# twndus/YelpRecommendation

Hardware: NVIDIA B200
Metric: ngcf_bpr_train_triples_per_sec (higher is better)
Workload: dtype f32

## Files before the change

### yelprecommendation_b200/csrc/common.cuh

```cuda
#pragma once
#include <cuda_runtime.h>
#include <cooperative_groups.h>
#include <stdint.h>
#include "../../include/yelprec_b200.h"

namespace cg = cooperative_groups;

#define YR_CHECK_LAUNCH()                                   \
  do {                                                      \
    cudaError_t e__ = cudaGetLastError();                   \
    if (e__ != cudaSuccess) return (int)e__;                \
  } while (0)

#define YR_CUDA(call)                                       \
  do {                                                      \
    cudaError_t e__ = (call);                               \
    if (e__ != cudaSuccess) return (int)e__;                \
  } while (0)

int yr_eval_exact_launch(const float* Uemb, int64_t nU, const float* Vt, int64_t ldt, int64_t nI, int d,
                         const int64_t* eval_uid, int64_t n_eval, const int32_t* mask_ptr,
                         const int32_t* mask_idx, const int32_t* act_ptr, const int32_t* act_idx,
                         const int32_t* act_nuniq, const double* inv_log2, int K, int64_t* topk_out,
                         float* topk_score, double* user_metrics, int32_t* err, const int32_t* row_list,
                         const int32_t* n_rows_dev, yr_stream stream, void* ws = nullptr, size_t ws_bytes = 0);
int yr_eval_reduce_launch(const double* user_metrics, const int32_t* act_ptr, const int32_t* act_nuniq,
                          int64_t n_eval, double* metric_sums, yr_stream stream);

int yr_ngcf_dense_fwd_tc_launch_d(int d, const float* E, const float* LE, const float* W1, const float* W2, float slope,
                                  int64_t n, float* Eout, cudaStream_t s, const int32_t* row_list = nullptr,
                                  const int32_t* row_count = nullptr, int64_t row_cap = 0, int reserve_sms = 0);
int yr_ngcf_dense_bwd_tc_launch(int d, const float* E, const float* LE, const float* En, const float* Gn, const float* W1,
                                const float* W2, float slope, int64_t n, float* G, float* T, float* ws, int* n_parts,
                                cudaStream_t s, const int32_t* row_list = nullptr, const int32_t* row_count = nullptr,
                                int64_t row_cap = 0, int reserve_sms = 0);
int yr_spmm_csr_rows(const yr_csr* A, int d, const float* X, float* Y, const int32_t* row_flag, cudaStream_t s);

namespace yr {

constexpr int kWarp = 32;
constexpr unsigned kFull = 0xffffffffu;

__device__ __forceinline__ float warp_sum(float v) {
#pragma unroll
  for (int o = 16; o > 0; o >>= 1) v += __shfl_xor_sync(kFull, v, o);
  return v;
}
__device__ __forceinline__ double warp_sum_d(double v) {
#pragma unroll
  for (int o = 16; o > 0; o >>= 1) v += __shfl_xor_sync(kFull, v, o);
  return v;
}

__device__ __forceinline__ void grid_sync(cg::grid_group& grid) {
  __syncwarp();
  grid.sync();
  __syncwarp();
}

template <int VPL> struct Row { float x[VPL]; };

template <int VPL>
__device__ __forceinline__ Row<VPL> ld_row(const float* __restrict__ row, int lane) {
  Row<VPL> r;
  if constexpr (VPL == 1) {
    r.x[0] = row[lane];
  } else if constexpr (VPL == 2) {
    float2 t = reinterpret_cast<const float2*>(row)[lane];
    r.x[0] = t.x; r.x[1] = t.y;
  } else {
#pragma unroll
    for (int j = 0; j < VPL / 4; ++j) {
      float4 t = reinterpret_cast<const float4*>(row)[j * 32 + lane];
      r.x[4 * j + 0] = t.x; r.x[4 * j + 1] = t.y; r.x[4 * j + 2] = t.z; r.x[4 * j + 3] = t.w;
    }
  }
  return r;
}

template <int VPL>
__device__ __forceinline__ Row<VPL> ld_row_cg(const float* __restrict__ row, int lane) {
  Row<VPL> r;
  if constexpr (VPL == 1) {
    r.x[0] = __ldcg(row + lane);
  } else if constexpr (VPL == 2) {
    float2 t = __ldcg(reinterpret_cast<const float2*>(row) + lane);
    r.x[0] = t.x; r.x[1] = t.y;
  } else {
// ... 151 lines not shown
```

### yelprecommendation_b200/csrc/ngcf.cu

```cuda
#include <stdlib.h>
#include "common.cuh"

namespace yr {

__device__ __forceinline__ void fma2(float2& acc, float a, const float2 b) { acc = __ffma2_rn(make_float2(a, a), b, acc); }

template <int D>
struct DenseCfg {
  static constexpr int kThreads = 256;
  static constexpr int kColGroups = D / 4;
  static constexpr int kRowGroups = kThreads / kColGroups;
  static constexpr int TM = 4 * kRowGroups;
  static constexpr int RO = D / kRowGroups;
  static constexpr size_t kSmemFwd = (size_t)(2 * D * TM + 2 * D * D) * sizeof(float);
  static constexpr size_t kSmemBwd = (size_t)(3 * TM * D + 2 * D * D) * sizeof(float);
  static_assert(D == 32 || D == 64 || D == 128, "dense transforms: D in {32, 64, 128}");
};

template <int D>
__global__ void __launch_bounds__(256)
ngcf_dense_fwd_kernel(const float* __restrict__ E, const float* __restrict__ LE,
                      const float* __restrict__ W1, const float* __restrict__ W2, float slope,
                      int64_t n, float* __restrict__ Eout) {
  using C = DenseCfg<D>;
// ... 406 lines not shown
                                 float* E_next, cudaStream_t s) {
  using C = DenseCfg<D>;
  static AttrOnce attr;
  { int rc_ = attr.set(ngcf_dense_fwd_kernel<D>, (int)C::kSmemFwd); if (rc_) return rc_; }
  const int64_t n_tiles = (n + C::TM - 1) / C::TM;
  int64_t grid = (int64_t)yr_sm_count() * (D <= 64 ? 3 : 1);
  if (grid > n_tiles) grid = n_tiles;
  ngcf_dense_fwd_kernel<D><<<(unsigned)grid, C::kThreads, C::kSmemFwd, s>>>(E, LE, W1, W2, slope, n, E_next);
  YR_CHECK_LAUNCH();
  return YR_OK;
}

template <int D>
static int dense_bwd_fp32_launch(int64_t n, const float* E, const float* LE, const float* E_next, const float* G_next,
                                 const float* W1, const float* W2, float slope, float* G, float* T, float* ws,
                                 cudaStream_t s, int* n_parts) {
  using C = DenseCfg<D>;
  static AttrOnce attr;
  { int rc_ = attr.set(ngcf_dense_bwd_kernel<D>, (int)C::kSmemBwd); if (rc_) return rc_; }
  const int64_t n_tiles = (n + C::TM - 1) / C::TM;
  int64_t grid = (int64_t)yr_sm_count() * (D <= 64 ? kBwdCtasPerSm : 1);
  if (grid > n_tiles) grid = n_tiles;
  ngcf_dense_bwd_kernel<D><<<(unsigned)grid, C::kThreads, C::kSmemBwd, s>>>(E, LE, E_next, G_next, W1, W2, slope, n, G, T, ws,
                                                                          nullptr, nullptr);
  YR_CHECK_LAUNCH();
  *n_parts = (int)grid;
  return YR_OK;
}

extern "C" int yr_ngcf_dense_fwd(int d, int64_t n, const float* E, const float* LE, const float* W1, const float* W2,
                                 float slope, float* E_next, int dense_mode, yr_stream stream) {
  if (!E || !LE || !W1 || !W2 || !E_next || n < 0 || !mode_ok(dense_mode)) return YR_ERR_BAD_ARG;
  if (d != 32 && d != 64 && d != 128) return YR_ERR_BAD_DIM;
  if (n == 0) return YR_OK;
  if (fwd_tc(dense_mode) && (d == 64 || d == 128))
    return yr_ngcf_dense_fwd_tc_launch_d(d, E, LE, W1, W2, slope, n, E_next, (cudaStream_t)stream, nullptr, nullptr, 0,
                                         reserve_of(dense_mode));
  switch (d) {
    case 32: return dense_fwd_fp32_launch<32>(n, E, LE, W1, W2, slope, E_next, (cudaStream_t)stream);
    case 64: return dense_fwd_fp32_launch<64>(n, E, LE, W1, W2, slope, E_next, (cudaStream_t)stream);
    default: return dense_fwd_fp32_launch<128>(n, E, LE, W1, W2, slope, E_next, (cudaStream_t)stream);
  }
}

extern "C" int yr_ngcf_layer_fwd(const yr_csr* L, int d, const float* E, const float* W1, const float* W2,
                                 float slope, float* E_next, float* LE_save, int dense_mode, yr_stream stream) {
  if (!L || !E || !W1 || !W2 || !E_next || !LE_save || L->n_rows <= 0 || !mode_ok(dense_mode)) return YR_ERR_BAD_ARG;
  if (d != 32 && d != 64 && d != 128) return YR_ERR_BAD_DIM;
  int rc = yr_spmm_csr(L, d, E, LE_save, 0, stream);
  if (rc) return rc;
  return yr_ngcf_dense_fwd(d, L->n_rows, E, LE_save, W1, W2, slope, E_next, dense_mode, stream);
}

extern "C" size_t yr_ngcf_layer_bwd_ws_bytes(int d) {
  return (size_t)yr_sm_count() * kBwdCtasPerSm * 2 * (size_t)d * d * sizeof(float);
}

static int dense_bwd_launch(int d, int64_t n, const float* E, const float* LE, const float* E_next, const float* G_next,
                            const float* W1, const float* W2, float slope, float* G, float* T, void* ws, size_t ws_bytes,
                            int dense_mode, cudaStream_t s, int* n_parts) {
  if (!E || !LE || !E_next || !G_next || !W1 || !W2 || !G || !T || !ws || n <= 0 || !mode_ok(dense_mode)) return YR_ERR_BAD_ARG;
  if (d != 32 && d != 64 && d != 128) return YR_ERR_BAD_DIM;
  if (ws_bytes < yr_ngcf_layer_bwd_ws_bytes(d)) return YR_ERR_WORKSPACE;
  if (bwd_tc(dense_mode) && (d == 64 || d == 128))
    return yr_ngcf_dense_bwd_tc_launch(d, E, LE, E_next, G_next, W1, W2, slope, n, G, T, (float*)ws, n_parts, s, nullptr, nullptr,
                                       0, reserve_of(dense_mode));
  switch (d) {
    case 32: return dense_bwd_fp32_launch<32>(n, E, LE, E_next, G_next, W1, W2, slope, G, T, (float*)ws, s, n_parts);
    case 64: return dense_bwd_fp32_launch<64>(n, E, LE, E_next, G_next, W1, W2, slope, G, T, (float*)ws, s, n_parts);
    default: return dense_bwd_fp32_launch<128>(n, E, LE, E_next, G_next, W1, W2, slope, G, T, (float*)ws, s, n_parts);
  }
}

static int dense_bwd_reduce(int d, const void* ws, int n_parts, float* dW1, float* dW2, cudaStream_t s) {
  const int len = 2 * d * d;
  reduce_partials_kernel<<<(len + 31) / 32, 256, 0, s>>>((const float*)ws, n_parts, len, dW1, dW2, d * d);
  YR_CHECK_LAUNCH();
  return YR_OK;
}

extern "C" int yr_ngcf_dense_bwd(int d, int64_t n, const float* E, const float* LE, const float* E_next,
                                 const float* G_next, const float* W1, const float* W2, float slope,
                                 float* G, float* T, float* dW1, float* dW2, void* ws, size_t ws_bytes,
                                 int dense_mode, yr_stream stream) {
  if (!dW1 || !dW2) return YR_ERR_BAD_ARG;
  int parts = 0;
  int rc = dense_bwd_launch(d, n, E, LE, E_next, G_next, W1, W2, slope, G, T, ws, ws_bytes, dense_mode, (cudaStream_t)stream,
                            &parts);
  if (rc) return rc;
  return dense_bwd_reduce(d, ws, parts, dW1, dW2, (cudaStream_t)stream);
}

namespace yr {
__global__ void __launch_bounds__(256)
touched_rows_kernel(const int64_t* __restrict__ uid, const int64_t* __restrict__ pos, const int64_t* __restrict__ neg,
                    int64_t B, int64_t nU, int64_t nI, int32_t* flag, int32_t* list, int32_t* count) {
  for (int64_t i = (int64_t)blockIdx.x * blockDim.x + threadIdx.x; i < 3 * B; i += (int64_t)gridDim.x * blockDim.x) {
    const int which = (int)(i / B);
    const int64_t b = i - which * B;
    const int64_t id = which == 0 ? uid[b] : (which == 1 ? pos[b] : neg[b]);
    if (id < 0 || id >= (which == 0 ? nU : nI)) continue;
    const int64_t row = which == 0 ? id : nU + id;
    if (atomicExch(flag + row, 1) == 0) list[atomicAdd(count, 1)] = (int32_t)row;
  }
}

__global__ void __launch_bounds__(256)
untouch_rows_kernel(int32_t* flag, const int32_t* __restrict__ list, const int32_t* __restrict__ count) {
  const int n = *count;
  for (int i = blockIdx.x * blockDim.x + threadIdx.x; i < n; i += gridDim.x * blockDim.x) flag[list[i]] = 0;
}

template <int D>
__global__ void __launch_bounds__(256)
spmm_scatter_rows_kernel(yr_csr A, const int32_t* __restrict__ flag, const float* __restrict__ T, float* __restrict__ G) {
  constexpr int kVec = D / 4, LPR = kVec >= 32 ? 32 : kVec, VPT = kVec / LPR, CPW = 32 / LPR;
  const int lane = threadIdx.x & 31, sub = lane / LPR, sl = lane % LPR;
  const int gwarp = (blockIdx.x * blockDim.x + threadIdx.x) >> 5;
  const int nwarps = (gridDim.x * blockDim.x) >> 5;
// ... 2 lines not shown
    const int c = cb + sub;
    int4 dsc = make_int4(0, 0, 0, -1);
    if (c < A.n_chunks) dsc = __ldg(desc + c);
    const int row = dsc.x, s0 = dsc.y;
    int len = dsc.z & 0xff;
    if (c >= A.n_chunks || !__ldg(flag + row)) len = 0;
    int maxlen = len;
#pragma unroll
    for (int o = LPR; o < 32; o <<= 1) maxlen = max(maxlen, __shfl_xor_sync(kFull, maxlen, o));
    if (maxlen == 0) continue;
    float4 t[VPT];
#pragma unroll
    for (int v = 0; v < VPT; ++v)
      t[v] = len ? reinterpret_cast<const float4*>(T + (int64_t)row * D)[sl * VPT + v] : make_float4(0.f, 0.f, 0.f, 0.f);
    for (int j0 = 0; j0 < maxlen; j0 += LPR) {
      const int j = j0 + sl;
      const int cc = (j < len) ? __ldg(A.col + s0 + j) : -1;
      const float aa = (j < len) ? __ldg(A.val + s0 + j) : 0.f;
      for (int q = 0; q < LPR && j0 + q < maxlen; ++q) {
        const int cq = __shfl_sync(kFull, cc, q, LPR);
        const float a = __shfl_sync(kFull, aa, q, LPR);
        if (cq >= 0) {
#pragma unroll
          for (int v = 0; v < VPT; ++v)
            atomicAdd(reinterpret_cast<float4*>(G + (int64_t)cq * D) + sl * VPT + v,
                      make_float4(a * t[v].x, a * t[v].y, a * t[v].z, a * t[v].w));
        }
      }
    }
  }
}
}

struct SideStream { cudaStream_t stream; cudaEvent_t fork, join; };
static SideStream* side_stream() {
  static SideStream pool[64];
  static int state[64];
  const char* e = getenv("YR_NGCF_SIDE_STREAM");
  if (e && e[0] == '0') return nullptr;
  int dev = 0;
  if (cudaGetDevice(&dev) != cudaSuccess || dev < 0 || dev >= 64) return nullptr;
  if (state[dev] == 0) {
    SideStream& x = pool[dev];
    const bool ok = cudaStreamCreateWithFlags(&x.stream, cudaStreamNonBlocking) == cudaSuccess &&
                    cudaEventCreateWithFlags(&x.fork, cudaEventDisableTiming) == cudaSuccess &&
                    cudaEventCreateWithFlags(&x.join, cudaEventDisableTiming) == cudaSuccess;
    state[dev] = ok ? 1 : -1;
  }
  return state[dev] == 1 ? &pool[dev] : nullptr;
}

static int rows_reduce(const yr_ngcf_state* st, int l, int parts, cudaStream_t s, SideStream* side);

static int ngcf_layer_bwd_rows(const yr_ngcf_state* st, int l, float slope, cudaStream_t s, SideStream* side) {
  const int d = st->d;
  using C = DenseCfg<64>;
  if (d != 64) return YR_ERR_BAD_DIM;
  if (bwd_tc(st->dense_mode) && st->row_list_cap >= 16384) {
    int parts = 0;
    int rc = yr_ngcf_dense_bwd_tc_launch(d, st->E[l], st->LE[l], st->E[l + 1], st->G[l + 1], st->W1[l], st->W2[l], slope,
                                         st->nU + st->nI, st->G[l], st->T, (float*)st->ws, &parts, s, st->row_list,
                                         st->row_count, st->row_list_cap);
    if (rc) return rc;
    rc = rows_reduce(st, l, parts, s, side);
    if (rc) return rc;
    const int64_t blocks_tc = ((int64_t)st->L.n_chunks + 15) / 16;
    spmm_scatter_rows_kernel<64><<<(unsigned)blocks_tc, 256, 0, s>>>(st->L, st->row_flag, st->T, st->G[l]);
    YR_CHECK_LAUNCH();
    return YR_OK;
  }
  int64_t grid = (st->row_list_cap + C::TM - 1) / C::TM;
  const int64_t cap = (int64_t)yr_sm_count() * kBwdCtasPerSm;
  if (grid > cap) grid = cap;
  if (grid < 1) grid = 1;
  static AttrOnce attr;
  { int rc_ = attr.set(ngcf_dense_bwd_kernel<64>, (int)C::kSmemBwd); if (rc_) return rc_; }
  ngcf_dense_bwd_kernel<64><<<(unsigned)grid, C::kThreads, C::kSmemBwd, s>>>(
      st->E[l], st->LE[l], st->E[l + 1], st->G[l + 1], st->W1[l], st->W2[l], slope, st->nU + st->nI, st->G[l], st->T,
      (float*)st->ws, st->row_list, st->row_count);
  YR_CHECK_LAUNCH();
  int rc = rows_reduce(st, l, (int)grid, s, side);
  if (rc) return rc;
  const int wpb = 8, cpw = 2;
  int64_t blocks = ((int64_t)st->L.n_chunks + wpb * cpw - 1) / (wpb * cpw);
  spmm_scatter_rows_kernel<64><<<(unsigned)blocks, 256, 0, s>>>(st->L, st->row_flag, st->T, st->G[l]);
  YR_CHECK_LAUNCH();
  return YR_OK;
}

static int rows_reduce(const yr_ngcf_state* st, int l, int parts, cudaStream_t s, SideStream* side) {
  const int len = 2 * st->d * st->d;
  cudaStream_t rs = s;
  if (side) {
    YR_CUDA(cudaEventRecord(side->fork, s));
    YR_CUDA(cudaStreamWaitEvent(side->stream, side->fork, 0));
    rs = side->stream;
  }
  reduce_partials_kernel<<<(len + 31) / 32, 256, 0, rs>>>((const float*)st->ws, parts, len, st->dW1[l], st->dW2[l],
                                                         st->d * st->d);
  YR_CHECK_LAUNCH();
  if (side) YR_CUDA(cudaEventRecord(side->join, side->stream));
  return YR_OK;
}

extern "C" int yr_ngcf_layer_bwd(const yr_csr* LT, int d, const float* E, const float* LE, const float* E_next,
                                 const float* G_next, const float* W1, const float* W2, float slope,
                                 float* G, float* T, float* dW1, float* dW2, void* ws, size_t ws_bytes,
                                 int dense_mode, yr_stream stream) {
  if (!LT || LT->n_rows <= 0) return YR_ERR_BAD_ARG;
  int rc = yr_ngcf_dense_bwd(d, LT->n_rows, E, LE, E_next, G_next, W1, W2, slope, G, T, dW1, dW2, ws, ws_bytes, dense_mode,
                             stream);
  if (rc) return rc;
  return yr_spmm_csr(LT, d, T, G, 1, stream);
// ... 96 lines not shown
  if (rc) return rc;
  if (n_prefix < 0 || n_prefix > st->n_layers) return YR_ERR_BAD_ARG;
  for (int l = 0; l < n_prefix; ++l) {
    rc = yr_ngcf_layer_fwd(&st->L, st->d, st->E[l], st->W1[l], st->W2[l], slope, st->E[l + 1], st->LE[l], st->dense_mode,
                           stream);
    if (rc) return rc;
  }
  return YR_OK;
}

extern "C" int yr_ngcf_propagate(const yr_ngcf_state* st, float slope, yr_stream stream) {
  int rc = ngcf_state_ok(st);
  if (rc) return rc;
  for (int l = 0; l < st->n_layers; ++l) {
    rc = yr_ngcf_layer_fwd(&st->L, st->d, st->E[l], st->W1[l], st->W2[l], slope,
                           st->E[l + 1], st->LE[l], st->dense_mode, stream);
    if (rc) return rc;
  }
  return YR_OK;
}

extern "C" int yr_ngcf_train_step_ex(const yr_ngcf_state* st, const yr_opt* opt, float slope,
                                     const int64_t* uid, const int64_t* pos, const int64_t* neg, int64_t B,
                                     float* step_loss, int prefix_done, yr_stream stream);

extern "C" int yr_ngcf_train_step(const yr_ngcf_state* st, const yr_opt* opt, float slope,
                                  const int64_t* uid, const int64_t* pos, const int64_t* neg, int64_t B,
                                  float* step_loss, yr_stream stream) {
  return yr_ngcf_train_step_ex(st, opt, slope, uid, pos, neg, B, step_loss, 0, stream);
}

static int train_step_body(const yr_ngcf_state* st, const yr_opt* opt, float slope,
                           const int64_t* uid, const int64_t* pos, const int64_t* neg, int64_t B,
                           float* step_loss, int prefix_done, yr_stream stream, bool* rows_armed) {
  int rc = ngcf_state_ok(st);
  if (rc) return rc;
  if (prefix_done < 0 || prefix_done > st->n_layers) return YR_ERR_BAD_ARG;
  if (!opt || !uid || !pos || !neg || B <= 0 || yr_csr_ok(&st->LT) || !st->T ||
      !st->E_dev || !st->G_dev || !st->ws || !st->loss)
    return YR_ERR_BAD_ARG;
  if (opt->kind < YR_OPT_SGD || opt->kind > YR_OPT_ADAMW) return YR_ERR_BAD_OPT;
  const int L = st->n_layers, d = st->d;
  const int64_t n = st->nU + st->nI;
  cudaStream_t s = (cudaStream_t)stream;
  SideStream* side = side_stream();
  for (int l = 0; l <= L; ++l)
    if (!st->G[l]) return YR_ERR_BAD_ARG;
  cudaStream_t ms = side ? side->stream : s;
  if (side) {
    YR_CUDA(cudaEventRecord(side->fork, s));
    YR_CUDA(cudaStreamWaitEvent(side->stream, side->fork, 0));
  }
  for (int l = 0; l <= L; ++l) YR_CUDA(cudaMemsetAsync(st->G[l], 0, sizeof(float) * (size_t)n * d, ms));
  const bool rows_path = st->row_flag && st->row_list && st->row_count && st->row_list_cap >= 3 * B && d == 64 &&
                         st->top_rows_mode != 0;
  if (rows_path) {
    touched_rows_kernel<<<(unsigned)((3 * B + 255) / 256), 256, 0, ms>>>(uid, pos, neg, B, st->nU, st->nI, st->row_flag,
                                                                        st->row_list, st->row_count);
    YR_CHECK_LAUNCH();
    *rows_armed = true;
  }
  if (side) YR_CUDA(cudaEventRecord(side->join, side->stream));
  if (rows_path && fwd_tc(st->dense_mode)) {
    for (int l = (prefix_done < L - 1 ? prefix_done : L - 1); l + 1 < L; ++l) {
      rc = yr_ngcf_layer_fwd(&st->L, d, st->E[l], st->W1[l], st->W2[l], slope, st->E[l + 1], st->LE[l], st->dense_mode,
                           stream);
      if (rc) return rc;
    }
    if (side) YR_CUDA(cudaStreamWaitEvent(s, side->join, 0));
    rc = yr_spmm_csr_rows(&st->L, d, st->E[L - 1], st->LE[L - 1], st->row_flag, s);
    if (rc) return rc;
    rc = yr_ngcf_dense_fwd_tc_launch_d(d, st->E[L - 1], st->LE[L - 1], st->W1[L - 1], st->W2[L - 1], slope, n, st->E[L], s,
                                       st->row_list, st->row_count, 3 * B);
    if (rc) return rc;
  } else {
    for (int l = prefix_done; l < L; ++l) {
      rc = yr_ngcf_layer_fwd(&st->L, d, st->E[l], st->W1[l], st->W2[l], slope, st->E[l + 1], st->LE[l], st->dense_mode,
                           stream);
      if (rc) return rc;
    }
  }
  if (side) YR_CUDA(cudaStreamWaitEvent(s, side->join, 0));
  rc = yr_ngcf_tail(st->E_dev, st->G_dev, L, st->nU, st->nI, d, uid, pos, neg, B, nullptr, nullptr, st->loss,
                    step_loss, st->err, stream);
  if (rc) return rc;
  bool reduce_pending = false;
  for (int l = L - 1; l >= 0; --l) {
    if (!st->dW1[l] || !st->dW2[l]) return YR_ERR_BAD_ARG;
    if (rows_path && l == L - 1) {
      rc = ngcf_layer_bwd_rows(st, l, slope, s, side);
      if (rc) return rc;
      reduce_pending = side != nullptr;
      cudaStream_t us = s;
      if (side) {
        YR_CUDA(cudaStreamWaitEvent(s, side->join, 0));
        reduce_pending = false;
        YR_CUDA(cudaEventRecord(side->fork, s));
        YR_CUDA(cudaStreamWaitEvent(side->stream, side->fork, 0));
        us = side->stream;
      }
      untouch_rows_kernel<<<(unsigned)((3 * B + 255) / 256), 256, 0, us>>>(st->row_flag, st->row_list, st->row_count);
      YR_CHECK_LAUNCH();
      YR_CUDA(cudaMemsetAsync(st->row_count, 0, sizeof(int32_t), us));
      *rows_armed = false;
      continue;
    }
    if (side && reduce_pending) { YR_CUDA(cudaStreamWaitEvent(s, side->join, 0)); reduce_pending = false; }
    int parts = 0;
    rc = dense_bwd_launch(d, n, st->E[l], st->LE[l], st->E[l + 1], st->G[l + 1], st->W1[l], st->W2[l], slope, st->G[l],
                          st->T, st->ws, st->ws_bytes, st->dense_mode, s, &parts);
    if (rc) return rc;
    if (side) {
      YR_CUDA(cudaEventRecord(side->fork, s));
      YR_CUDA(cudaStreamWaitEvent(side->stream, side->fork, 0));
      rc = dense_bwd_reduce(d, st->ws, parts, st->dW1[l], st->dW2[l], side->stream);
      if (rc) return rc;
      YR_CUDA(cudaEventRecord(side->join, side->stream));
      reduce_pending = true;
    } else {
      rc = dense_bwd_reduce(d, st->ws, parts, st->dW1[l], st->dW2[l], s);
      if (rc) return rc;
    }
    rc = yr_spmm_csr(&st->LT, d, st->T, st->G[l], 1, stream);
    if (rc) return rc;
  }
  if (side && reduce_pending) YR_CUDA(cudaStreamWaitEvent(s, side->join, 0));
  float *pp[2 * YR_NGCF_MAX_LAYERS + 1], *gg[2 * YR_NGCF_MAX_LAYERS + 1], *mm[2 * YR_NGCF_MAX_LAYERS + 1],
      *vv[2 * YR_NGCF_MAX_LAYERS + 1];
  int64_t nn[2 * YR_NGCF_MAX_LAYERS + 1];
  int cnt = 0;
  pp[cnt] = st->E[0]; gg[cnt] = st->G[0]; mm[cnt] = st->mE; vv[cnt] = st->vE; nn[cnt++] = n * d;
  for (int l = 0; l < L; ++l) {
    pp[cnt] = st->W1[l]; gg[cnt] = st->dW1[l]; mm[cnt] = st->mW1[l]; vv[cnt] = st->vW1[l]; nn[cnt++] = (int64_t)d * d;
    pp[cnt] = st->W2[l]; gg[cnt] = st->dW2[l]; mm[cnt] = st->mW2[l]; vv[cnt] = st->vW2[l]; nn[cnt++] = (int64_t)d * d;
  }
  for (int c0 = 0; c0 < cnt; c0 += YR_OPT_MAX_TENSORS) {
    const int c = (cnt - c0 < YR_OPT_MAX_TENSORS) ? cnt - c0 : YR_OPT_MAX_TENSORS;
    rc = yr_dense_opt_step_multi(c, pp + c0, gg + c0, mm + c0, vv + c0, nn + c0, opt, 0, stream);
    if (rc) return rc;
  }
  return YR_OK;
}

extern "C" int yr_ngcf_train_step_ex(const yr_ngcf_state* st, const yr_opt* opt, float slope,
                                     const int64_t* uid, const int64_t* pos, const int64_t* neg, int64_t B,
                                     float* step_loss, int prefix_done, yr_stream stream) {
  bool rows_armed = false;
  const int rc = train_step_body(st, opt, slope, uid, pos, neg, B, step_loss, prefix_done, stream, &rows_armed);
  if (rc == YR_OK) return rc;
  cudaStream_t s = (cudaStream_t)stream;
  if (SideStream* side = side_stream()) {
    if (cudaEventRecord(side->join, side->stream) == cudaSuccess) cudaStreamWaitEvent(s, side->join, 0);
  }
  if (rows_armed && st && st->row_flag && st->row_list && st->row_count) {
    untouch_rows_kernel<<<(unsigned)((3 * B + 255) / 256), 256, 0, s>>>(st->row_flag, st->row_list, st->row_count);
    cudaMemsetAsync(st->row_count, 0, sizeof(int32_t), s);
  }
  return rc;
}

extern "C" int yr_ngcf_concat(const float* const* E_layers, int n_layers, int64_t n, int d, float* out,
                              yr_stream stream) {
  if (!E_layers || !out || n <= 0 || d <= 0 || (d & 3) || n_layers < 0 || n_layers > YR_NGCF_MAX_LAYERS)
// ... 9 lines not shown
```

### yelprecommendation_b200/csrc/ngcf_tc_bwd.cu

```cuda
#include <stdlib.h>
#include "tc_common.cuh"

namespace yr {

constexpr int kBwdThreads = 416;
constexpr int kBwdTM = 128;
constexpr int kFlushTiles = 4;

__device__ __forceinline__ uint32_t mn_off(int mn, int k, uint32_t lbo, uint32_t sbo) {
  return (uint32_t)(k >> 2) * sbo + (uint32_t)(mn >> 5) * lbo + (uint32_t)(k & 3) * 128u +
         ((((uint32_t)(mn & 31) >> 3) ^ (uint32_t)(k & 3)) << 5) + (uint32_t)(mn & 7) * 4u;
}
__device__ __forceinline__ uint64_t mn_desc(uint32_t smem_addr, uint32_t lbo, uint32_t sbo) {
  uint64_t d = 0;
  d |= (uint64_t)((smem_addr & 0x3FFFFu) >> 4);
  d |= (uint64_t)((lbo >> 4) & 0x3FFFu) << 16;
  d |= (uint64_t)((sbo >> 4) & 0x3FFFu) << 32;
  d |= (uint64_t)1 << 46;
  d |= (uint64_t)1 << 61;
  return d;
}
__device__ __forceinline__ void mbar_expect_tx_b(uint64_t* bar, uint32_t bytes) {
  asm volatile("mbarrier.expect_tx.relaxed.cta.shared::cta.b64 [%0], %1;" ::"r"(s2u(bar)), "r"(bytes) : "memory");
}
__device__ __forceinline__ void bulk_g2s_b(void* dst, const void* src, uint32_t bytes, uint64_t* bar) {
  asm volatile("cp.async.bulk.shared::cluster.global.mbarrier::complete_tx::bytes [%0], [%1], %2, [%3];" ::"r"(s2u(dst)),
               "l"(src), "r"(bytes), "r"(s2u(bar))
               : "memory");
}

template <int D>
struct BwdTc {
  static_assert(D == 64 || D == 128, "tensor-core backward: d in {64, 128}");
  static constexpr int kSlabs = D / 32;
  static constexpr int kXG = D == 128 ? 2 : 1;
  static constexpr int kHalves = D / 64;
  static constexpr uint32_t kBlk = 16384;
  static constexpr uint32_t kPair = 2 * kBlk;
  static constexpr uint32_t kStage = (1 + kXG) * kPair;
  static constexpr int kNst = D == 128 ? 2 : 3;
  static constexpr uint32_t kRing = kNst * kStage;
  static constexpr uint32_t kEpiOff = kRing;
  static constexpr uint32_t kEpiBytes = 4 * 32 * 256;
  static constexpr uint32_t kBarOff = kEpiOff + kEpiBytes;
  static constexpr size_t kSmem = (size_t)kBarOff + 256 + 1024;
  static constexpr int kAcc = D == 128 ? 1 : 2;
  static constexpr uint32_t kAccCols = D == 128 ? 256 : 128;
  static constexpr uint32_t kTmemCols = 512;
  static constexpr uint32_t kColG2 = 256;
  static constexpr uint32_t kSboW = 2048, kSboSP = 2048, kSboZ = (D / 32) * 512, kLbo = 512;
  static constexpr int kItems = kSlabs + 4 * kHalves;
  static constexpr size_t kWsplitBytes = (size_t)kSlabs * kXG * kPair;
};

template <int D>
__global__ void __launch_bounds__(256)
ngcf_split_weights_bwd_kernel(const float* __restrict__ W1, const float* __restrict__ W2, unsigned char* __restrict__ ws) {
  using C = BwdTc<D>;
  const int total = 2 * D * (D / 4);
  for (int idx = blockIdx.x * blockDim.x + threadIdx.x; idx < total; idx += gridDim.x * blockDim.x) {
    const int X = idx / (D * (D / 4)), rem = idx % (D * (D / 4));
    const int o = rem / (D / 4), c4 = rem % (D / 4), j = o >> 5, k = o & 31;
    float4 hi, lo;
    split4(__ldg(reinterpret_cast<const float4*>((X ? W2 : W1) + o * D) + c4), hi, lo);
    const int pair = C::kXG == 2 ? X : 0;
    const int mn = C::kXG == 2 ? 4 * c4 : X * D + 4 * c4;
    unsigned char* blk = ws + (size_t)(j * C::kXG + pair) * C::kPair;
    const uint32_t off = mn_off(mn, k, C::kLbo, C::kSboW);
    *reinterpret_cast<float4*>(blk + off) = hi;
    *reinterpret_cast<float4*>(blk + C::kBlk + off) = lo;
  }
}

template <int D>
__global__ void __launch_bounds__(kBwdThreads, 1)
ngcf_dense_bwd_tc_kernel(const float* __restrict__ E, const float* __restrict__ LE, const float* __restrict__ Enext,
                         const float* __restrict__ Gnext, const unsigned char* __restrict__ wsplit, float slope, int64_t n,
                         float* __restrict__ G, float* __restrict__ T, float* __restrict__ ws,
                         const int32_t* __restrict__ row_list, const int32_t* __restrict__ row_count) {
  using C = BwdTc<D>;
  constexpr int TM = kBwdTM, kNst = C::kNst, kXG = C::kXG, kSlabs = C::kSlabs, kHalves = C::kHalves, kItems = C::kItems;
  constexpr uint32_t kBlk = C::kBlk, kPair = C::kPair, kStage = C::kStage;
  if (row_list) n = *row_count;
  extern __shared__ __align__(16) unsigned char smem_raw[];
  unsigned char* smem = smem_raw + ((1024u - (s2u(smem_raw) & 1023u)) & 1023u);
  unsigned char* ring = smem;
  uint64_t* bars = reinterpret_cast<uint64_t*>(smem + C::kBarOff);
  uint64_t* full = bars; uint64_t* empty = bars + kNst; uint64_t* d1_full = bars + 2 * kNst; uint64_t* d1_empty = d1_full + 2;
  uint64_t* d2_full = d1_full + 4; uint64_t* d2_empty = d1_full + 5;
  uint32_t* tmem_slot = reinterpret_cast<uint32_t*>(d1_full + 6);
  constexpr int kAcc = C::kAcc;

  const int tid = threadIdx.x, lane = tid & 31, warp = tid >> 5;
  const int64_t n_tiles = (n + TM - 1) / TM;
  const int64_t my_tiles = (int64_t)blockIdx.x < n_tiles ? (n_tiles - blockIdx.x + gridDim.x - 1) / gridDim.x : 0;

  if (tid == 0) {
    for (int s = 0; s < kNst; ++s) { mbar_init(full + s, 1); mbar_init(empty + s, 1); }
    for (int a = 0; a < 2; ++a) { mbar_init(d1_full + a, 1); mbar_init(d1_empty + a, 128); }
    mbar_init(d2_full, 1); mbar_init(d2_empty, 128);
    asm volatile("fence.mbarrier_init.release.cluster;" ::: "memory");
  }
  if (warp == 12) tmem_alloc(tmem_slot, C::kTmemCols);
  tc_fence_before();
  __syncthreads();
  tc_fence_after();
  const uint32_t tmem_base = *tmem_slot;
  const uint32_t idesc1 = (1u << 4) | (2u << 7) | (2u << 10) | (1u << 16) | ((uint32_t)(128 >> 3) << 17) | ((uint32_t)(128 >> 4) << 24);
  const uint32_t idesc2 = (1u << 4) | (2u << 7) | (2u << 10) | (1u << 15) | (1u << 16) | ((uint32_t)(D >> 3) << 17) |
                          ((uint32_t)(128 >> 4) << 24);

  if (warp < 8) {
// ... 214 lines not shown
          const uint32_t a[2] = {st, st + kBlk}, b[2] = {st + (1 + x) * kPair, st + (1 + x) * kPair + kBlk};
          const int pa[3] = {1, 0, 0}, pb[3] = {0, 1, 0};
#pragma unroll
          for (int p = 0; p < 3; ++p) {
            const uint64_t ad = sw128_desc(a[pa[p]]);
#pragma unroll
            for (int ks = 0; ks < 4; ++ks) {
              const uint64_t bd = mn_desc(b[pb[p]] + (uint32_t)(ks * 2) * C::kSboW, C::kLbo, C::kSboW);
              umma_tf32(tmem_base + acc * C::kAccCols + x * 128, ad + 2 * ks, bd, idesc1, (j == 0 && p == 0 && ks == 0) ? 0u : 1u);
            }
          }
        }
        umma_commit(empty + s);
        if (++s == (uint32_t)kNst) { s = 0; ph ^= 1; }
      }
      umma_commit(d1_full + acc);
      if (t > 0 && t % kFlushTiles == 0) {
        mbar_wait(d2_empty, n_flush & 1);
        ++n_flush;
        tc_fence_after();
        first2 = 1;
      }
#pragma unroll 1
      for (int q = 0; q < 4; ++q) {
        mbar_wait(full + s, ph);
        tc_fence_after();
        const uint32_t st = s2u(ring + (size_t)s * kStage);
#pragma unroll
        for (int x = 0; x < kXG; ++x) {
          const uint32_t a[2] = {st + (1 + x) * kPair, st + (1 + x) * kPair + kBlk}, b[2] = {st, st + kBlk};
          const int pa[3] = {1, 0, 0}, pb[3] = {0, 1, 0};
#pragma unroll
          for (int p = 0; p < 3; ++p) {
#pragma unroll
            for (int ks = 0; ks < 4; ++ks) {
              const uint64_t ad = mn_desc(a[pa[p]] + (uint32_t)(ks * 2) * C::kSboSP, C::kLbo, C::kSboSP);
              const uint64_t bd = mn_desc(b[pb[p]] + (uint32_t)(ks * 2) * C::kSboZ, C::kLbo, C::kSboZ);
              umma_tf32(tmem_base + C::kColG2 + x * 128, ad, bd, idesc2, (first2 && p == 0 && ks == 0) ? 0u : 1u);
            }
          }
        }
        first2 = 0;
        umma_commit(empty + s);
        if (++s == (uint32_t)kNst) { s = 0; ph ^= 1; }
      }
      if ((t + 1) % kFlushTiles == 0 || t + 1 == my_tiles) umma_commit(d2_full);
    }
  }
  tc_fence_before();
  __syncthreads();
  if (warp == 12) tmem_dealloc(tmem_base, C::kTmemCols);
}

}

using namespace yr;

template <int D>
static int bwd_tc_launch(const float* E, const float* LE, const float* En, const float* Gn, const float* W1, const float* W2,
                         float slope, int64_t n, float* G, float* T, float* ws, int* n_parts, cudaStream_t s,
                         const int32_t* row_list, const int32_t* row_count, int64_t row_cap, int reserve_sms) {
  using C = BwdTc<D>;
  static yr::AttrOnce attr;
  { int rc_ = attr.set(ngcf_dense_bwd_tc_kernel<D>, (int)C::kSmem); if (rc_) return rc_; }
  const int64_t n_tiles = ((row_list ? row_cap : n) + kBwdTM - 1) / kBwdTM;
  const int64_t sms = yr_sm_count();
  int64_t grid = sms - reserve_sms;
  if (grid > n_tiles) grid = n_tiles;
  if (grid < 1) grid = 1;
  unsigned char* wsplit = reinterpret_cast<unsigned char*>(ws) + (size_t)sms * 2 * D * D * sizeof(float);
  ngcf_split_weights_bwd_kernel<D><<<16, 256, 0, s>>>(W1, W2, wsplit);
  YR_CHECK_LAUNCH();
  ngcf_dense_bwd_tc_kernel<D><<<(unsigned)grid, kBwdThreads, C::kSmem, s>>>(E, LE, En, Gn, wsplit, slope, n, G, T, ws, row_list,
                                                                            row_count);
  YR_CHECK_LAUNCH();
  *n_parts = (int)grid;
  return YR_OK;
}

int yr_ngcf_dense_bwd_tc_launch(int d, const float* E, const float* LE, const float* En, const float* Gn, const float* W1,
                                const float* W2, float slope, int64_t n, float* G, float* T, float* ws, int* n_parts,
                                cudaStream_t s, const int32_t* row_list, const int32_t* row_count, int64_t row_cap,
                                int reserve_sms) {
  if (d == 64) return bwd_tc_launch<64>(E, LE, En, Gn, W1, W2, slope, n, G, T, ws, n_parts, s, row_list, row_count, row_cap, reserve_sms);
  if (d == 128) return bwd_tc_launch<128>(E, LE, En, Gn, W1, W2, slope, n, G, T, ws, n_parts, s, row_list, row_count, row_cap, reserve_sms);
  return YR_ERR_BAD_DIM;
}
```

Measured before the change: 3.967 million.

## Add specialized d=64 tcgen05 dense backward kernel and batch weight splitting per step

```diff
diff --git a/yelprecommendation_b200/csrc/common.cuh b/yelprecommendation_b200/csrc/common.cuh
--- a/yelprecommendation_b200/csrc/common.cuh
+++ b/yelprecommendation_b200/csrc/common.cuh
@@ -30,10 +30,13 @@
 int yr_ngcf_dense_fwd_tc_launch_d(int d, const float* E, const float* LE, const float* W1, const float* W2, float slope,
                                   int64_t n, float* Eout, cudaStream_t s, const int32_t* row_list = nullptr,
                                   const int32_t* row_count = nullptr, int64_t row_cap = 0, int reserve_sms = 0);
-int yr_ngcf_dense_bwd_tc_launch(int d, const float* E, const float* LE, const float* En, const float* Gn, const float* W1,
-                                const float* W2, float slope, int64_t n, float* G, float* T, float* ws, int* n_parts,
-                                cudaStream_t s, const int32_t* row_list = nullptr, const int32_t* row_count = nullptr,
-                                int64_t row_cap = 0, int reserve_sms = 0);
+int yr_ngcf_dense_bwd_tc_launch(int d, const float* E, const float* LE, const float* En, const float* Gn,
+                                const unsigned char* wsplit, float slope, int64_t n, float* G, float* T, float* ws,
+                                int* n_parts, cudaStream_t s, const int32_t* row_list = nullptr,
+                                const int32_t* row_count = nullptr, int64_t row_cap = 0, int reserve_sms = 0);
+size_t yr_ngcf_bwd_wsplit_bytes(int d);
+int yr_ngcf_split_weights_bwd_launch(int d, int n_layers, const float* const* W1, const float* const* W2, unsigned char* out,
+                                     cudaStream_t s);
 int yr_spmm_csr_rows(const yr_csr* A, int d, const float* X, float* Y, const int32_t* row_flag, cudaStream_t s);
 
 namespace yr {
diff --git a/yelprecommendation_b200/csrc/ngcf.cu b/yelprecommendation_b200/csrc/ngcf.cu
--- a/yelprecommendation_b200/csrc/ngcf.cu
+++ b/yelprecommendation_b200/csrc/ngcf.cu
@@ -482,19 +482,28 @@
   return yr_ngcf_dense_fwd(d, L->n_rows, E, LE_save, W1, W2, slope, E_next, dense_mode, stream);
 }
 
+static size_t bwd_partials_bytes(int d) { return (size_t)yr_sm_count() * kBwdCtasPerSm * 2 * (size_t)d * d * sizeof(float); }
+
 extern "C" size_t yr_ngcf_layer_bwd_ws_bytes(int d) {
-  return (size_t)yr_sm_count() * kBwdCtasPerSm * 2 * (size_t)d * d * sizeof(float);
+  return bwd_partials_bytes(d) + (size_t)YR_NGCF_MAX_LAYERS * yr_ngcf_bwd_wsplit_bytes(d);
 }
 
 static int dense_bwd_launch(int d, int64_t n, const float* E, const float* LE, const float* E_next, const float* G_next,
                             const float* W1, const float* W2, float slope, float* G, float* T, void* ws, size_t ws_bytes,
-                            int dense_mode, cudaStream_t s, int* n_parts) {
+                            int dense_mode, cudaStream_t s, int* n_parts, const unsigned char* wsplit = nullptr) {
   if (!E || !LE || !E_next || !G_next || !W1 || !W2 || !G || !T || !ws || n <= 0 || !mode_ok(dense_mode)) return YR_ERR_BAD_ARG;
   if (d != 32 && d != 64 && d != 128) return YR_ERR_BAD_DIM;
   if (ws_bytes < yr_ngcf_layer_bwd_ws_bytes(d)) return YR_ERR_WORKSPACE;
-  if (bwd_tc(dense_mode) && (d == 64 || d == 128))
-    return yr_ngcf_dense_bwd_tc_launch(d, E, LE, E_next, G_next, W1, W2, slope, n, G, T, (float*)ws, n_parts, s, nullptr, nullptr,
-                                       0, reserve_of(dense_mode));
+  if (bwd_tc(dense_mode) && (d == 64 || d == 128)) {
+    if (!wsplit) {
+      unsigned char* own = (unsigned char*)ws + (size_t)yr_sm_count() * 2 * d * d * sizeof(float);
+      int rc = yr_ngcf_split_weights_bwd_launch(d, 1, &W1, &W2, own, s);
+      if (rc) return rc;
+      wsplit = own;
+    }
+    return yr_ngcf_dense_bwd_tc_launch(d, E, LE, E_next, G_next, wsplit, slope, n, G, T, (float*)ws, n_parts, s, nullptr,
+                                       nullptr, 0, reserve_of(dense_mode));
+  }
   switch (d) {
     case 32: return dense_bwd_fp32_launch<32>(n, E, LE, E_next, G_next, W1, W2, slope, G, T, (float*)ws, s, n_parts);
     case 64: return dense_bwd_fp32_launch<64>(n, E, LE, E_next, G_next, W1, W2, slope, G, T, (float*)ws, s, n_parts);
@@ -603,13 +612,17 @@
 
 static int rows_reduce(const yr_ngcf_state* st, int l, int parts, cudaStream_t s, SideStream* side);
 
+static const unsigned char* step_wsplit(const yr_ngcf_state* st, int l) {
+  return (const unsigned char*)st->ws + bwd_partials_bytes(st->d) + (size_t)l * yr_ngcf_bwd_wsplit_bytes(st->d);
+}
+
 static int ngcf_layer_bwd_rows(const yr_ngcf_state* st, int l, float slope, cudaStream_t s, SideStream* side) {
   const int d = st->d;
   using C = DenseCfg<64>;
   if (d != 64) return YR_ERR_BAD_DIM;
   if (bwd_tc(st->dense_mode) && st->row_list_cap >= 16384) {
     int parts = 0;
-    int rc = yr_ngcf_dense_bwd_tc_launch(d, st->E[l], st->LE[l], st->E[l + 1], st->G[l + 1], st->W1[l], st->W2[l], slope,
+    int rc = yr_ngcf_dense_bwd_tc_launch(d, st->E[l], st->LE[l], st->E[l + 1], st->G[l + 1], step_wsplit(st, l), slope,
                                          st->nU + st->nI, st->G[l], st->T, (float*)st->ws, &parts, s, st->row_list,
                                          st->row_count, st->row_list_cap);
     if (rc) return rc;
@@ -812,6 +825,12 @@
     YR_CUDA(cudaStreamWaitEvent(side->stream, side->fork, 0));
   }
   for (int l = 0; l <= L; ++l) YR_CUDA(cudaMemsetAsync(st->G[l], 0, sizeof(float) * (size_t)n * d, ms));
+  const bool tc_bwd = bwd_tc(st->dense_mode) && (d == 64 || d == 128);
+  if (tc_bwd) {
+    if (st->ws_bytes < yr_ngcf_layer_bwd_ws_bytes(d)) return YR_ERR_WORKSPACE;
+    rc = yr_ngcf_split_weights_bwd_launch(d, L, st->W1, st->W2, (unsigned char*)step_wsplit(st, 0), ms);
+    if (rc) return rc;
+  }
   const bool rows_path = st->row_flag && st->row_list && st->row_count && st->row_list_cap >= 3 * B && d == 64 &&
                          st->top_rows_mode != 0;
   if (rows_path) {
@@ -868,7 +887,7 @@
     if (side && reduce_pending) { YR_CUDA(cudaStreamWaitEvent(s, side->join, 0)); reduce_pending = false; }
     int parts = 0;
     rc = dense_bwd_launch(d, n, st->E[l], st->LE[l], st->E[l + 1], st->G[l + 1], st->W1[l], st->W2[l], slope, st->G[l],
-                          st->T, st->ws, st->ws_bytes, st->dense_mode, s, &parts);
+                          st->T, st->ws, st->ws_bytes, st->dense_mode, s, &parts, tc_bwd ? step_wsplit(st, l) : nullptr);
     if (rc) return rc;
     if (side) {
       YR_CUDA(cudaEventRecord(side->fork, s));
diff --git a/yelprecommendation_b200/csrc/ngcf_tc_bwd.cu b/yelprecommendation_b200/csrc/ngcf_tc_bwd.cu
--- a/yelprecommendation_b200/csrc/ngcf_tc_bwd.cu
+++ b/yelprecommendation_b200/csrc/ngcf_tc_bwd.cu
@@ -53,11 +53,16 @@
   static constexpr size_t kWsplitBytes = (size_t)kSlabs * kXG * kPair;
 };
 
+struct BwdWeights { const float* W1[YR_NGCF_MAX_LAYERS]; const float* W2[YR_NGCF_MAX_LAYERS]; };
+
 template <int D>
 __global__ void __launch_bounds__(256)
-ngcf_split_weights_bwd_kernel(const float* __restrict__ W1, const float* __restrict__ W2, unsigned char* __restrict__ ws) {
+ngcf_split_weights_bwd_kernel(const __grid_constant__ BwdWeights w, unsigned char* __restrict__ ws) {
   using C = BwdTc<D>;
   const int total = 2 * D * (D / 4);
+  const float* W1 = w.W1[blockIdx.y];
+  const float* W2 = w.W2[blockIdx.y];
+  ws += (size_t)blockIdx.y * C::kWsplitBytes;
   for (int idx = blockIdx.x * blockDim.x + threadIdx.x; idx < total; idx += gridDim.x * blockDim.x) {
     const int X = idx / (D * (D / 4)), rem = idx % (D * (D / 4));
     const int o = rem / (D / 4), c4 = rem % (D / 4), j = o >> 5, k = o & 31;
@@ -378,37 +383,311 @@
   if (warp == 12) tmem_dealloc(tmem_base, C::kTmemCols);
 }
 
+struct Bwd64 {
+  using C = BwdTc<64>;
+  static constexpr int kNst = 2;
+  static constexpr uint32_t kStage = 2 * C::kPair;
+  static constexpr uint32_t kZk = 8192;
+  static constexpr uint32_t kWOff = 0;
+  static constexpr uint32_t kRingOff = (uint32_t)C::kWsplitBytes;
+  static constexpr uint32_t kEpiOff = kRingOff + kNst * kStage;
+  static constexpr uint32_t kEpiBuf = 32 * 128 * 4;
+  static constexpr uint32_t kBarOff = kEpiOff + 2 * kEpiBuf;
+  static constexpr size_t kSmem = (size_t)kBarOff + 256 + 1024;
+};
+
+__global__ void __launch_bounds__(kBwdThreads, 1)
+ngcf_dense_bwd_tc64_kernel(const float* __restrict__ E, const float* __restrict__ LE, const float* __restrict__ Enext,
+                           const float* __restrict__ Gnext, const unsigned char* __restrict__ wsplit, float slope, int64_t n,
+                           float* __restrict__ G, float* __restrict__ T, float* __restrict__ ws,
+                           const int32_t* __restrict__ row_list, const int32_t* __restrict__ row_count) {
+  using C = BwdTc<64>;
+  using K = Bwd64;
+  constexpr int D = 64, TM = kBwdTM, kNst = K::kNst;
+  constexpr uint32_t kBlk = C::kBlk, kPair = C::kPair, kStage = K::kStage;
+  if (row_list) n = *row_count;
+  extern __shared__ __align__(16) unsigned char smem_raw[];
+  unsigned char* smem = smem_raw + ((1024u - (s2u(smem_raw) & 1023u)) & 1023u);
+  unsigned char* wsm = smem + K::kWOff;
+  unsigned char* ring = smem + K::kRingOff;
+  uint64_t* bars = reinterpret_cast<uint64_t*>(smem + K::kBarOff);
+  uint64_t* full = bars; uint64_t* empty = bars + kNst; uint64_t* d1_full = bars + 2 * kNst; uint64_t* d1_empty = d1_full + 2;
+  uint64_t* d2_full = d1_full + 4; uint64_t* d2_empty = d1_full + 5; uint64_t* wbar = d1_full + 6;
+  uint32_t* tmem_slot = reinterpret_cast<uint32_t*>(d1_full + 7);
+
+  const int tid = threadIdx.x, lane = tid & 31, warp = tid >> 5;
+  const int64_t n_tiles = (n + TM - 1) / TM;
+  const int64_t my_tiles = (int64_t)blockIdx.x < n_tiles ? (n_tiles - blockIdx.x + gridDim.x - 1) / gridDim.x : 0;
+
+  if (tid == 0) {
+    for (int s = 0; s < kNst; ++s) { mbar_init(full + s, 1); mbar_init(empty + s, 1); }
+    for (int a = 0; a < 2; ++a) { mbar_init(d1_full + a, 1); mbar_init(d1_empty + a, 128); }
+    mbar_init(d2_full, 1); mbar_init(d2_empty, 128); mbar_init(wbar, 1);
+    asm volatile("fence.mbarrier_init.release.cluster;" ::: "memory");
+  }
+  if (warp == 12) tmem_alloc(tmem_slot, C::kTmemCols);
+  tc_fence_before();
+  __syncthreads();
+  tc_fence_after();
+  const uint32_t tmem_base = *tmem_slot;
+  if (tid == 0 && my_tiles > 0) {
+    mbar_expect_tx(wbar, (uint32_t)C::kWsplitBytes);
+    bulk_g2s_b(wsm, wsplit, (uint32_t)C::kWsplitBytes, wbar);
+  }
+  const uint32_t idesc1 = (1u << 4) | (2u << 7) | (2u << 10) | (1u << 15) | ((uint32_t)(32 >> 3) << 17) | ((uint32_t)(128 >> 4) << 24);
+  const uint32_t idesc2 = (1u << 4) | (2u << 7) | (2u << 10) | (1u << 15) | (1u << 16) | ((uint32_t)(D >> 3) << 17) |
+                          ((uint32_t)(128 >> 4) << 24);
+
+  if (warp < 8) {
+    const int64_t n_items = my_tiles * 4;
+    uint32_t s = 0, ph = 0;
+    const int c4 = tid & 15, r0 = tid >> 4;
+    auto issue = [&](int64_t item, float4 (&x)[8]) {
+      const int64_t tile = blockIdx.x + (item >> 2) * gridDim.x;
+      const int qc = (int)(item & 3);
+#pragma unroll
+      for (int r = 0; r < 2; ++r) {
+        const int64_t q = tile * TM + 32 * qc + r0 + 16 * r;
+        x[r] = make_float4(0.f, 0.f, 0.f, 0.f); x[2 + r] = x[r]; x[4 + r] = x[r]; x[6 + r] = x[r];
+        if (q < n) {
+          const int64_t g = (row_list ? (int64_t)__ldg(row_list + q) : q) * (D / 4) + c4;
+          x[r] = __ldg(reinterpret_cast<const float4*>(Gnext) + g);
+          x[2 + r] = __ldg(reinterpret_cast<const float4*>(Enext) + g);
+          x[4 + r] = __ldg(reinterpret_cast<const float4*>(E) + g);
+          x[6 + r] = __ldg(reinterpret_cast<const float4*>(LE) + g);
+        }
+      }
+    };
+    auto process = [&](const float4 (&x)[8]) {
+      unsigned char* st = ring + (size_t)s * kStage;
+      mbar_wait(empty + s, ph ^ 1);
+#pragma unroll
+      for (int r = 0; r < 2; ++r) {
+        const int k = r0 + 16 * r;
+        const float4 g = x[r], en = x[2 + r], e = x[4 + r], le = x[6 + r];
+        float4 z, hi, lo;
+        z.x = en.x > 0.f ? g.x : g.x * slope; z.y = en.y > 0.f ? g.y : g.y * slope;
+        z.z = en.z > 0.f ? g.z : g.z * slope; z.w = en.w > 0.f ? g.w : g.w * slope;
+        split4(z, hi, lo);
+        const uint32_t oz = mn_off(4 * c4, k, C::kLbo, C::kSboZ);
+        *reinterpret_cast<float4*>(st + oz) = hi;
+        *reinterpret_cast<float4*>(st + kBlk + oz) = lo;
+        const uint32_t ok = K::kZk + sw_off(32, k, c4);
+        *reinterpret_cast<float4*>(st + ok) = hi;
+        *reinterpret_cast<float4*>(st + kBlk + ok) = lo;
+        split4(make_float4(le.x + e.x, le.y + e.y, le.z + e.z, le.w + e.w), hi, lo);
+        const uint32_t os = mn_off(4 * c4, k, C::kLbo, C::kSboSP);
+        *reinterpret_cast<float4*>(st + kPair + os) = hi;
+        *reinterpret_cast<float4*>(st + kPair + kBlk + os) = lo;
+        split4(make_float4(e.x * le.x, e.y * le.y, e.z * le.z, e.w * le.w), hi, lo);
+        const uint32_t op = mn_off(D + 4 * c4, k, C::kLbo, C::kSboSP);
+        *reinterpret_cast<float4*>(st + kPair + op) = hi;
+        *reinterpret_cast<float4*>(st + kPair + kBlk + op) = lo;
+      }
+      asm volatile("fence.proxy.async.shared::cta;" ::: "memory");
+      asm volatile("bar.sync 1, 256;" ::: "memory");
+      if (tid == 0) mbar_arrive(full + s);
+      if (++s == (uint32_t)kNst) { s = 0; ph ^= 1; }
+    };
+    float4 xa[8], xb[8];
+    if (n_items > 0) issue(0, xa);
+    for (int64_t it = 0; it < n_items; it += 2) {
+      if (it + 1 < n_items) issue(it + 1, xb);
+      process(xa);
+      if (it + 1 < n_items) {
+        if (it + 2 < n_items) issue(it + 2, xa);
+        process(xb);
+      }
+    }
+  } else if (warp < 12) {
+    const int wq = warp & 3;
+    const uint32_t lane_base = (uint32_t)(wq * 32) << 16;
+    uint32_t fph = 0;
+    bool flushed = false;
+    const int r = wq * 32 + lane;
+    auto drain_dw = [&]() {
+      float* my = ws + (size_t)blockIdx.x * 2 * D * D + (size_t)(r >> 6) * D * D + (r & 63);
+#pragma unroll 1
+      for (int c0 = 0; c0 < D; c0 += 16) {
+        float v[16];
+        tmem_ld16(tmem_base + lane_base + C::kColG2 + c0, v);
+        if (flushed) {
+#pragma unroll
+          for (int j = 0; j < 16; ++j) v[j] += my[(size_t)(c0 + j) * D];
+        }
+#pragma unroll
+        for (int j = 0; j < 16; ++j) my[(size_t)(c0 + j) * D] = v[j];
+      }
+    };
+    const int k = lane & 15, sub = lane >> 4;
+    for (int64_t t = 0; t < my_tiles; ++t) {
+      if (t > 0 && t % kFlushTiles == 0) {
+        mbar_wait(d2_full, fph);
+        fph ^= 1;
+        tc_fence_after();
+        drain_dw();
+        flushed = true;
+        tc_fence_before();
+        mbar_arrive(d2_empty);
+      }
+      const int acc = (int)(t & 1);
+      mbar_wait(d1_full + acc, (uint32_t)(t >> 1) & 1u);
+      tc_fence_after();
+#pragma unroll 1
+      for (int q = 0; q < 4; ++q) {
+        float* buf = reinterpret_cast<float*>(smem + K::kEpiOff + (q & 1) * K::kEpiBuf);
+        {
+          float v[32];
+          tmem_ld32(tmem_base + lane_base + acc * C::kAccCols + 32 * q, v);
+          if (q == 3) {
+            tc_fence_before();
+            mbar_arrive(d1_empty + acc);
+          }
+#pragma unroll
+          for (int j = 0; j < 32; ++j) buf[j * 128 + r] = v[j];
+        }
+        asm volatile("bar.sync 2, 128;" ::: "memory");
+        const int64_t q0 = (blockIdx.x + t * gridDim.x) * TM + 32 * q + 8 * wq;
+        float4 ev[4], lv[4], gv[4];
+        int64_t g4[4];
+#pragma unroll
+        for (int i = 0; i < 4; ++i) {
+          const int64_t qq = q0 + 2 * i + sub;
+          g4[i] = -1;
+          if (qq < n) {
+            g4[i] = (row_list ? (int64_t)__ldg(row_list + qq) : qq) * (D / 4) + k;
+            ev[i] = __ldg(reinterpret_cast<const float4*>(E) + g4[i]);
+            lv[i] = __ldg(reinterpret_cast<const float4*>(LE) + g4[i]);
+            gv[i] = *(reinterpret_cast<const float4*>(G) + g4[i]);
+          }
+        }
+#pragma unroll
+        for (int i = 0; i < 4; ++i) {
+          if (g4[i] < 0) continue;
+          const int rr = 8 * wq + 2 * i + sub;
+          const float4 ds = *reinterpret_cast<const float4*>(buf + rr * 128 + 4 * k);
+          const float4 dp = *reinterpret_cast<const float4*>(buf + rr * 128 + 64 + 4 * k);
+          float4 tt, gg = gv[i];
+          tt.x = fmaf(dp.x, ev[i].x, ds.x); tt.y = fmaf(dp.y, ev[i].y, ds.y);
+          tt.z = fmaf(dp.z, ev[i].z, ds.z); tt.w = fmaf(dp.w, ev[i].w, ds.w);
+          gg.x += fmaf(dp.x, lv[i].x, ds.x); gg.y += fmaf(dp.y, lv[i].y, ds.y);
+          gg.z += fmaf(dp.z, lv[i].z, ds.z); gg.w += fmaf(dp.w, lv[i].w, ds.w);
+          reinterpret_cast<float4*>(T)[g4[i]] = tt;
+          reinterpret_cast<float4*>(G)[g4[i]] = gg;
+        }
+      }
+    }
+    if (my_tiles > 0) {
+      mbar_wait(d2_full, fph);
+      tc_fence_after();
+      drain_dw();
+    } else {
+      for (int idx = r; idx < 2 * D * D; idx += 128) ws[(size_t)blockIdx.x * 2 * D * D + idx] = 0.f;
+    }
+  } else if (lane == 0) {
+    uint32_t s = 0, ph = 0, first2 = 1, n_flush = 0;
+    if (my_tiles > 0) mbar_wait(wbar, 0);
+    tc_fence_after();
+    const uint32_t w0 = s2u(wsm);
+    for (int64_t t = 0; t < my_tiles; ++t) {
+      const int acc = (int)(t & 1);
+      mbar_wait(d1_empty + acc, ((uint32_t)(t >> 1) & 1u) ^ 1u);
+      tc_fence_after();
+      if (t > 0 && t % kFlushTiles == 0) {
+        mbar_wait(d2_empty, n_flush & 1);
+        ++n_flush;
+        tc_fence_after();
+        first2 = 1;
+      }
+#pragma unroll 1
+      for (int q = 0; q < 4; ++q) {
+        mbar_wait(full + s, ph);
+        tc_fence_after();
+        const uint32_t st = s2u(ring + (size_t)s * kStage);
+#pragma unroll
+        for (int j = 0; j < 2; ++j) {
+#pragma unroll
+          for (int p = 0; p < 3; ++p) {
+            const uint32_t wa = w0 + (uint32_t)j * kPair + (p == 1 ? kBlk : 0u);
+            const uint64_t bd = sw128_desc(st + (p == 0 ? kBlk : 0u) + K::kZk + (uint32_t)j * 4096u);
+#pragma unroll
+            for (int ks = 0; ks < 4; ++ks) {
+              const uint64_t ad = mn_desc(wa + (uint32_t)(ks * 2) * C::kSboW, C::kLbo, C::kSboW);
+              umma_tf32(tmem_base + acc * C::kAccCols + 32 * q, ad, bd + 2 * ks, idesc1, (j == 0 && p == 0 && ks == 0) ? 0u : 1u);
+            }
+          }
+        }
+        const uint32_t a[2] = {st + kPair, st + kPair + kBlk}, b[2] = {st, st + kBlk};
+        const int pa[3] = {1, 0, 0}, pb[3] = {0, 1, 0};
+#pragma unroll
+        for (int p = 0; p < 3; ++p) {
+#pragma unroll
+          for (int ks = 0; ks < 4; ++ks) {
+            const uint64_t ad = mn_desc(a[pa[p]] + (uint32_t)(ks * 2) * C::kSboSP, C::kLbo, C::kSboSP);
+            const uint64_t bd = mn_desc(b[pb[p]] + (uint32_t)(ks * 2) * C::kSboZ, C::kLbo, C::kSboZ);
+            umma_tf32(tmem_base + C::kColG2, ad, bd, idesc2, (first2 && p == 0 && ks == 0) ? 0u : 1u);
+          }
+        }
+        first2 = 0;
+        umma_commit(empty + s);
+        if (++s == (uint32_t)kNst) { s = 0; ph ^= 1; }
+      }
+      umma_commit(d1_full + acc);
+      if ((t + 1) % kFlushTiles == 0 || t + 1 == my_tiles) umma_commit(d2_full);
+    }
+  }
+  tc_fence_before();
+  __syncthreads();
+  if (warp == 12) tmem_dealloc(tmem_base, C::kTmemCols);
+}
+
 }
 
 using namespace yr;
 
 template <int D>
-static int bwd_tc_launch(const float* E, const float* LE, const float* En, const float* Gn, const float* W1, const float* W2,
+static int bwd_tc_launch(const float* E, const float* LE, const float* En, const float* Gn, const unsigned char* wsplit,
                          float slope, int64_t n, float* G, float* T, float* ws, int* n_parts, cudaStream_t s,
                          const int32_t* row_list, const int32_t* row_count, int64_t row_cap, int reserve_sms) {
   using C = BwdTc<D>;
+  auto* kernel = [] { if constexpr (D == 64) return ngcf_dense_bwd_tc64_kernel; else return ngcf_dense_bwd_tc_kernel<D>; }();
+  constexpr size_t smem = [] { if constexpr (D == 64) return Bwd64::kSmem; else return C::kSmem; }();
   static yr::AttrOnce attr;
-  { int rc_ = attr.set(ngcf_dense_bwd_tc_kernel<D>, (int)C::kSmem); if (rc_) return rc_; }
+  { int rc_ = attr.set(kernel, (int)smem); if (rc_) return rc_; }
   const int64_t n_tiles = ((row_list ? row_cap : n) + kBwdTM - 1) / kBwdTM;
-  const int64_t sms = yr_sm_count();
-  int64_t grid = sms - reserve_sms;
+  int64_t grid = yr_sm_count() - reserve_sms;
   if (grid > n_tiles) grid = n_tiles;
   if (grid < 1) grid = 1;
-  unsigned char* wsplit = reinterpret_cast<unsigned char*>(ws) + (size_t)sms * 2 * D * D * sizeof(float);
-  ngcf_split_weights_bwd_kernel<D><<<16, 256, 0, s>>>(W1, W2, wsplit);
-  YR_CHECK_LAUNCH();
-  ngcf_dense_bwd_tc_kernel<D><<<(unsigned)grid, kBwdThreads, C::kSmem, s>>>(E, LE, En, Gn, wsplit, slope, n, G, T, ws, row_list,
-                                                                            row_count);
+  kernel<<<(unsigned)grid, kBwdThreads, smem, s>>>(E, LE, En, Gn, wsplit, slope, n, G, T, ws, row_list, row_count);
   YR_CHECK_LAUNCH();
   *n_parts = (int)grid;
   return YR_OK;
 }
 
-int yr_ngcf_dense_bwd_tc_launch(int d, const float* E, const float* LE, const float* En, const float* Gn, const float* W1,
-                                const float* W2, float slope, int64_t n, float* G, float* T, float* ws, int* n_parts,
-                                cudaStream_t s, const int32_t* row_list, const int32_t* row_count, int64_t row_cap,
-                                int reserve_sms) {
-  if (d == 64) return bwd_tc_launch<64>(E, LE, En, Gn, W1, W2, slope, n, G, T, ws, n_parts, s, row_list, row_count, row_cap, reserve_sms);
-  if (d == 128) return bwd_tc_launch<128>(E, LE, En, Gn, W1, W2, slope, n, G, T, ws, n_parts, s, row_list, row_count, row_cap, reserve_sms);
+size_t yr_ngcf_bwd_wsplit_bytes(int d) {
+  if (d == 64) return BwdTc<64>::kWsplitBytes;
+  if (d == 128) return BwdTc<128>::kWsplitBytes;
+  return 0;
+}
+
+int yr_ngcf_split_weights_bwd_launch(int d, int n_layers, const float* const* W1, const float* const* W2, unsigned char* out,
+                                     cudaStream_t s) {
+  if (n_layers < 1 || n_layers > YR_NGCF_MAX_LAYERS) return YR_ERR_BAD_ARG;
+  BwdWeights w{};
+  for (int l = 0; l < n_layers; ++l) { w.W1[l] = W1[l]; w.W2[l] = W2[l]; }
+  const dim3 grid(16, (unsigned)n_layers);
+  if (d == 64) ngcf_split_weights_bwd_kernel<64><<<grid, 256, 0, s>>>(w, out);
+  else if (d == 128) ngcf_split_weights_bwd_kernel<128><<<grid, 256, 0, s>>>(w, out);
+  else return YR_ERR_BAD_DIM;
+  YR_CHECK_LAUNCH();
+  return YR_OK;
+}
+
+int yr_ngcf_dense_bwd_tc_launch(int d, const float* E, const float* LE, const float* En, const float* Gn,
+                                const unsigned char* wsplit, float slope, int64_t n, float* G, float* T, float* ws,
+                                int* n_parts, cudaStream_t s, const int32_t* row_list, const int32_t* row_count,
+                                int64_t row_cap, int reserve_sms) {
+  if (d == 64) return bwd_tc_launch<64>(E, LE, En, Gn, wsplit, slope, n, G, T, ws, n_parts, s, row_list, row_count, row_cap, reserve_sms);
+  if (d == 128) return bwd_tc_launch<128>(E, LE, En, Gn, wsplit, slope, n, G, T, ws, n_parts, s, row_list, row_count, row_cap, reserve_sms);
   return YR_ERR_BAD_DIM;
 }
```

Result: faster. 4.046 million, median of 6 (+2.0%).
